# Samleo8/RadarSLAMPy

Measured on AMD Instinct MI355X. Metric: radar scan-pairs/sec (400x3768 polar), higher is better.
Workload: dtype u8/f32/f64

## Files before the change

### profiles/ri_prof.py

```python
#!/usr/bin/env python3
import ctypes as C, os, sys
sys.path.insert(0, os.path.dirname(os.path.dirname(os.path.abspath(__file__))))
import numpy as np
from radarslampy_amd import _ffi, synth
from radarslampy_amd.engine import Engine
os.environ["ROAM_LIB_PARTIAL"] = "1"
N = 512
recs, poses, feat = synth.make_sequence(5, 2, n_static=460, n_movers=24, distortion=True)
ctx = _ffi.Context(0)
eng = Engine(N, 2 * N, ctx=ctx, retrack_on_device=True, retrack_slots=N)
for t in range(2): eng.upload_scan(t, recs[t])
for b in range(1, N):
    for t in range(2): eng.copy_scan(b * 2 + t, t)
for b in range(N): eng.init_lane(b, b * 2, feat[:40], poses[0])
eng.set_retrack(2); eng.step(np.arange(N, dtype=np.int32) * 2 + 1); eng.synchronize()
lib = _ffi.load_library()
lib.roam_debug_integral_prof.argtypes = [C.c_void_p, C.c_int]
out = (C.c_ulonglong * 16)()
lib.roam_debug_integral_prof(out, 1)
ms, by = eng.time_kernel("doh_integral", 3)
lib.roam_debug_integral_prof(out, 0)
v = np.array(list(out), float)
names = ["col: loop head", "col: barrier wait", "col: C (tile -> HBM)", "col: A1 (box + taps)", "col: A2 (column sums -> tile)", "row: loop head", "row: barrier wait", "row: B = rest"]
print(f"doh_integral {ms:.2f} ms per {N}")
tot_c = v[:5].sum()
for k in range(5): print(f"  {names[k]:32s} {100 * v[k] / tot_c:5.1f} %")
tot_r = v[8 + 5] + v[8 + 6]
print(f"  row wave: loop body (B + head) {100 * v[8 + 5] / tot_r:5.1f} %   barrier wait {100 * v[8 + 6] / tot_r:5.1f} %")
eng.close(); ctx.close()
```

### radarslampy_amd/csrc/engine.hip

```cpp
#include "roam_internal.h"
#include "retrack.h"
#include "kabsch_body.inc"
#include <algorithm>
#include <new>

#define KS ROAM_MAX_FEATURES
#define CART_CENTER 1012.0
#define M_PER_PX 0.0864
#define N_RETRACK 60
#define ROT_THR 0.2
#define TRANS_THR_SQ 4.0
#define ERR_THR 10.0f
#define TWO_PI 6.283185307179586476925286766559

#define RES_RING 8
enum { ST_PEAKS = 0, ST_WARP, ST_PYR, ST_KLT, ST_GRAPH, ST_CLIQUE, ST_KABSCH, ST_LM, ST_GLUE, ST_RETRACK, ST_COUNT };
static const char *kStageNames[ST_COUNT] = {"ingest_peaks", "warp_quantise", "pyramid", "klt", "consistency_graph",
                                            "max_clique", "kabsch", "mds_lm", "glue", "retrack"};

struct Engine {
    roam_engine_cfg cfg;
    int B = 0, W = 0, stage_cap = 0;
    PyrDesc pd;
    size_t rec_bytes = 0;
// ... 691 lines not shown
            return ROAM_E_HIP;
        }
        RtArgs &r = e->rt;
        r.pool = e->pool; r.map = e->warp_map; r.feat = e->feat; r.feat_n = e->feat_n; r.vel = e->vel; r.kf_und = e->kf_und; r.res = nullptr;
    }
    for (auto &ev : e->ev_res)
        if (hipEventCreateWithFlags(&ev, hipEventDisableTiming) != hipSuccess) { ROAM_SET_ERR(ctx, "hipEventCreate failed"); roam_engine_destroy(ctx); return ROAM_E_HIP; }
    e->slot_seq.assign((size_t)cfg->pool_scans, 0);
    for (auto &ev : e->ev_up_ring)
        if (hipEventCreateWithFlags(&ev, hipEventDisableTiming) != hipSuccess) { ROAM_SET_ERR(ctx, "hipEventCreate failed"); roam_engine_destroy(ctx); return ROAM_E_HIP; }
    if (hipEventCreateWithFlags(&e->ev_pool, hipEventDisableTiming) != hipSuccess) {
        ROAM_SET_ERR(ctx, "hipEventCreate failed"); roam_engine_destroy(ctx); return ROAM_E_HIP;
    }
    for (auto &ev : e->ev) {
        if (hipEventCreate(&ev) != hipSuccess) { ROAM_SET_ERR(ctx, "hipEventCreate failed"); roam_engine_destroy(ctx); return ROAM_E_HIP; }
    }
    if (hipEventCreate(&e->ev_join) != hipSuccess ||
        hipEventCreate(&e->ev_pk0) != hipSuccess || hipEventCreate(&e->ev_pk1) != hipSuccess ||
        hipEventCreateWithFlags(&e->ev_warp, hipEventDisableTiming) != hipSuccess || hipEventCreateWithFlags(&e->ev_idx, hipEventDisableTiming) != hipSuccess ||
        hipEventCreateWithFlags(&e->ev_peaks, hipEventDisableTiming) != hipSuccess) {
        ROAM_SET_ERR(ctx, "hipEventCreate failed"); roam_engine_destroy(ctx); return ROAM_E_HIP;
    }
    for (int i = 0; i < 4; i++)
        if (hipEventCreateWithFlags(&e->ev_klt[i], hipEventDisableTiming) != hipSuccess || hipEventCreateWithFlags(&e->ev_g4[i], hipEventDisableTiming) != hipSuccess) {
            ROAM_SET_ERR(ctx, "hipEventCreate failed"); roam_engine_destroy(ctx); return ROAM_E_HIP;
        }
    e->ev_ok = true;
    e->tr_ok = true;
    HIP_TRY(ctx, launch_warp_map(ctx->stream, cfg->rows, cfg->clip, e->warp_map));
    HIP_TRY(ctx, launch_pyr_dark(ctx->stream, e->warp_map, e->W, e->W, cfg->clip, e->pyr_dark));
    if (e->rt_on) HIP_TRY(ctx, launch_retrack_boxtab(ctx->stream, e->warp_map, e->W, cfg->clip, const_cast<uint32_t *>(e->rt.boxtab)));
    if (e->rt_on) HIP_TRY(ctx, launch_retrack_darktab(ctx->stream, e->warp_map, e->W, cfg->clip, const_cast<uint32_t *>(e->rt.darktab)));
    if (e->rt_on && e->rt.fused) { const int32_t rc_ = fused_tables(ctx, e); if (rc_ != ROAM_OK) { roam_engine_destroy(ctx); return rc_; } }
    HIP_TRY(ctx, hipStreamSynchronize(ctx->stream));
    e->rt_image_px = (int64_t)e->W * e->W;
    if (e->rt_on && e->W <= 2048 && B >= RT_TWO_PASS_SLOTS) {
        e->rt_image_px = 0;
        const size_t npx = (size_t)e->W * e->W, ndt = retrack_darktab_words(e->W), nph = retrack_phase_words(e->W);
        uint32_t *stage = nullptr;
        HIP_TRY(ctx, hipHostMalloc(reinterpret_cast<void **>(&stage), (npx + ndt + nph) * 4, hipHostMallocDefault));
        uint32_t *mh = stage, *dh = stage + npx;
        std::vector<uint32_t> ph(nph, 0u);
        hipError_t ec = hipMemcpyAsync(mh, e->warp_map, npx * 4, hipMemcpyDeviceToHost, ctx->stream);
        if (ec == hipSuccess) ec = hipMemcpyAsync(dh, e->rt.darktab, ndt * 4, hipMemcpyDeviceToHost, ctx->stream);
        if (ec == hipSuccess) ec = hipStreamSynchronize(ctx->stream);
        bool okp = ec == hipSuccess && retrack_build_phases(mh, dh, e->W, cfg->clip, ph.data());
        if (okp) {
            memcpy(stage + npx + ndt, ph.data(), nph * 4);
            ec = hipMemcpyAsync(const_cast<uint32_t *>(e->rt.phlist), stage + npx + ndt, nph * 4, hipMemcpyHostToDevice, ctx->stream);
            if (ec == hipSuccess) ec = hipStreamSynchronize(ctx->stream);
        }
        (void)hipHostFree(stage);
        if (!okp || ec != hipSuccess) { ROAM_SET_ERR(ctx, "retrack: phase list (%s)", ec != hipSuccess ? hipGetErrorString(ec) : "image too large"); roam_engine_destroy(ctx); return ec != hipSuccess ? ROAM_E_HIP : ROAM_E_ARG; }
        for (uint32_t i = 0; i < ph[0]; i++) {
            const int br = retrack_band_rows(), band = (int)(ph[1 + i] & 255u), g = (int)((ph[1 + i] >> 8) & 15u), hrows = std::min(br, e->W - br * band);
            for (int w = 0; w < 4; w++)
                if ((ph[1 + i] >> (12 + w)) & 1u) e->rt_image_px += (int64_t)hrows * std::max(0, std::min(64, e->W - (g * 256 + 64 * w)));
        }
    }
    return ROAM_OK;
}

#define ENGINE()                                  \
    if (!ctx) return ROAM_E_ARG;                  \
    Engine *e = ctx->engine;                      \
    if (!e) { ROAM_SET_ERR(ctx, "engine not created"); return ROAM_E_STATE; } \
    HIP_TRY(ctx, hipSetDevice(ctx->device))

int32_t roam_engine_upload_scan(roam_ctx *ctx, int32_t pool_idx, const uint8_t *rec)
{
    ENGINE();
    ARG_CHECK(ctx, rec && pool_idx >= 0 && pool_idx < e->cfg.pool_scans);
    e->slot_writes[(size_t)pool_idx]++;
    HIP_TRY(ctx, hipMemcpyAsync(e->pool + (size_t)pool_idx * e->rec_bytes, rec, e->rec_bytes, hipMemcpyHostToDevice, ctx->stream));
    HIP_TRY(ctx, hipStreamSynchronize(ctx->stream));
    return ROAM_OK;
}

int32_t roam_engine_upload_scans_async(roam_ctx *ctx, int32_t pool_idx0, int32_t n, const uint8_t *host_records, int64_t host_stride)
{
    ENGINE();
    ARG_CHECK(ctx, host_records && n >= 1 && pool_idx0 >= 0 && pool_idx0 + n <= e->cfg.pool_scans && (host_stride == 0 || host_stride >= (int64_t)e->rec_bytes));
    hipPointerAttribute_t at;
    const hipError_t pa = hipPointerGetAttributes(&at, host_records);
    if (pa != hipSuccess || (at.type != hipMemoryTypeHost && at.type != hipMemoryTypeManaged && at.type != hipMemoryTypeDevice)) {
        (void)hipGetLastError();
        ROAM_SET_ERR(ctx, "upload_scans_async: host_records is not pinned host memory (hipHostMalloc / hipHostRegister / roam_host_alloc)");
        return ROAM_E_ARG;
    }
    const uint8_t *dev_alias = at.devicePointer ? static_cast<const uint8_t *>(at.devicePointer) : host_records;
    const int width = e->cfg.payload_off + e->cfg.clip;
    hipLaunchKernelGGL(ingest_rows_kernel, dim3((e->cfg.rows + 3) / 4, n), dim3(256), 0, ctx->stream3, dev_alias, host_stride,
                       e->pool + (size_t)pool_idx0 * e->rec_bytes, (int64_t)e->rec_bytes, e->cfg.rows, e->cfg.stride, width);
    HIP_TRY(ctx, hipGetLastError());
    HIP_TRY(ctx, hipEventRecord(ctx->ev_up, ctx->stream3));
    e->up_seq++;
    for (int i = 0; i < n; i++) { e->slot_seq[(size_t)pool_idx0 + i] = e->up_seq; e->slot_writes[(size_t)pool_idx0 + i]++; }
    HIP_TRY(ctx, hipEventRecord(e->ev_up_ring[e->up_seq & 15], ctx->stream3));
    e->uploads_pending = true;
    return ROAM_OK;
}

int32_t roam_engine_fence(roam_ctx *ctx)
{
    ENGINE();
    HIP_TRY(ctx, hipEventRecord(ctx->ev_fence, ctx->stream));
    HIP_TRY(ctx, hipStreamWaitEvent(ctx->stream3, ctx->ev_fence, 0));
    return ROAM_OK;
}

int32_t roam_engine_copy_scan(roam_ctx *ctx, int32_t dst_idx, int32_t src_idx)
// ... 1012 lines not shown
```

### radarslampy_amd/csrc/retrack.h

```cpp
#pragma once
#include "roam_internal.h"
#include "blobprune.h"

#define RT_TWO_PASS_SLOTS 200
enum { RT_F_CAND_OVERFLOW = 1, RT_F_TREE_OVERFLOW = 2, RT_F_PAIR_OVERFLOW = 4, RT_F_FEAT_OVERFLOW = 8 };

struct RtArgs {
    int W, rows, cols, stride, payload_off, slots, size1, size2;
    int64_t rec_bytes;
    double sigma1, sigma2, threshold;
    const uint8_t *pool;
    const uint32_t *map;
    const uint32_t *phlist;
    const uint32_t *boxtab;
    const uint32_t *darktab;
    float *feat;
    int32_t *feat_n;
    const double *vel;
    double *kf_und;
    roam_lane_result *res;
    int32_t *rt_n, *rt_lane, *rt_scan;
    double *S;
    int32_t *col_done;
    double *colT;
    int SP;
    uint32_t *cand_rc;
    double *cand_val;
    int32_t *cand_n;
    BpTask *tasks;
    uint32_t *pairs;
    uint16_t *order;
    uint32_t *ovbits;
    uint16_t *bigtab;
    double *kp;
    int32_t *kp_n, *slot_flags;
    int32_t *ssc_work;
    int32_t *sel, *sel_n;
    int32_t *blob_order_buf;
    const int32_t *blob_order;
    int fused;
    const uint32_t *fd_mapT;
    const uint32_t *fd_boxtab;
    const uint32_t *fd_darktab;
    double *fd_halo;
    int64_t fd_halo_words;
    double *fd_cc;
};

hipError_t launch_retrack_collect(hipStream_t st, const roam_lane_result *res, const int32_t *scan_idx, int B, int force_all, const RtArgs &a);
#define RT_TRACE_CHUNKS 16
struct RtSide { hipStream_t st; hipEvent_t ev_i[4], ev_d[4]; int chunk; };
bool retrack_sided(const RtArgs &a, int B, const RtSide *side);
hipError_t launch_retrack(hipStream_t st, const RtArgs &a, int B, hipEvent_t *trace = nullptr, int ntrace = 0, hipEvent_t after_order = nullptr, const RtSide *side = nullptr);
hipError_t launch_ssc_batch(hipStream_t st, const double *kp, int64_t kp_stride, const int32_t *count, int kp_cap, int P,
                            int num_ret, double tol, int cols, int rows, int32_t *work, int32_t *sel, int32_t *n_sel,
                            const int32_t *n_active, int first);
hipError_t launch_retrack_part(hipStream_t st, const RtArgs &a, int P, int which);
hipError_t launch_retrack_emit(hipStream_t st, const RtArgs &a, int P);
hipError_t retrack_init();
size_t retrack_boxtab_words(int W);
size_t retrack_phase_words(int W);
int retrack_band_rows();
bool retrack_build_phases(const uint32_t *map_host, const uint32_t *darktab_host, int W, int cols, uint32_t *out);
hipError_t launch_retrack_boxtab(hipStream_t st, const uint32_t *map, int W, int cols, uint32_t *boxtab);
size_t retrack_darktab_words(int W);
size_t retrack_fused_boxtab_words(int W);
size_t retrack_fused_halo_words(int W);
hipError_t launch_retrack_fused_tables(hipStream_t st, const uint32_t *map, int W, int cols, uint32_t *mapT, uint32_t *boxtab, uint32_t *darktab);
hipError_t launch_retrack_darktab(hipStream_t st, const uint32_t *map, int W, int cols, uint32_t *darktab);
```

### radarslampy_amd/csrc/retrack_integral.hip

```cpp
#include "retrack_geom.h"

#define RT_TWO_PASS_Z 8
#define RC_BAND 64
#define RC_Q 16
__global__ __launch_bounds__(256) void rt_integ_cols_kernel(RtArgs a, int first, int P)
{
    const int nls = rt_one_sweep(a, first) ? 0 : min(min(RT_TWO_PASS_SLOTS, P), *a.rt_n - first);
    if ((int)blockIdx.z >= nls) return;
    __shared__ double tot[4][64];
    __shared__ float lut[256];
    __shared__ int last_s;
    lut[threadIdx.x] = rt_code_to_f32(threadIdx.x);
    const int lane = threadIdx.x & 63, q = threadIdx.x >> 6;
    const int c = blockIdx.x * 64 + lane, W = a.W, band = blockIdx.y, nb = (W + RC_BAND - 1) / RC_BAND;
    for (int ls = blockIdx.z; ls < nls; ls += (int)gridDim.z) {
    const int slot = first + ls;
    const uint8_t *p = a.pool + (int64_t)a.rt_scan[slot] * a.rec_bytes + a.payload_off;
    double *S = a.S + (int64_t)ls * a.SP * W;
    const int rows = a.rows, cols = a.cols, stride = a.stride;
    const int r0 = band * RC_BAND + q * RC_Q;
    uint32_t m[RC_Q];
#pragma unroll
    for (int k = 0; k < RC_Q; k++) m[k] = (c < W && r0 + k < W) ? a.map[(int64_t)(r0 + k) * W + c] : 0xfffu;
    __syncthreads();
// ... 69 lines not shown
    double acc = 0;
    auto step = [&](double2 (&x)[8], double2 &o, int i) {
        const int c = i * RR_COLS + lc;
#pragma unroll
        for (int k = 0; k < 8; k++) {
            const bool rin = r0 + 2 * k + lr < H;
            *reinterpret_cast<double2 *>(&tile[2 * k + lr][lc]) =
                make_double2(rin && c < W ? __dadd_rn(x[k].x, o.x) : 0.0, rin && c + 1 < W ? __dadd_rn(x[k].y, o.y) : 0.0);
        }
        fetch(x, o, min(i + RR_DEPTH, ntiles - 1));
        __syncthreads();
        if (threadIdx.x < RR_ROWS) {
            double2 *row = reinterpret_cast<double2 *>(tile[threadIdx.x]);
            double2 y[8], z[8];
#pragma unroll
            for (int j = 0; j < 8; j++) y[j] = row[j];
            for (int j0 = 0; j0 < RR_COLS / 2; j0 += 16) {
#pragma unroll
                for (int j = 0; j < 8; j++) z[j] = row[j0 + 8 + j];
#pragma unroll
                for (int j = 0; j < 8; j++) { acc = __dadd_rn(acc, y[j].x); y[j].x = acc; acc = __dadd_rn(acc, y[j].y); y[j].y = acc; }
#pragma unroll
                for (int j = 0; j < 8; j++) row[j0 + j] = y[j];
                const int jn = min(j0 + 16, RR_COLS / 2 - 8);
#pragma unroll
                for (int j = 0; j < 8; j++) y[j] = row[jn + j];
#pragma unroll
                for (int j = 0; j < 8; j++) { acc = __dadd_rn(acc, z[j].x); z[j].x = acc; acc = __dadd_rn(acc, z[j].y); z[j].y = acc; }
#pragma unroll
                for (int j = 0; j < 8; j++) row[j0 + 8 + j] = z[j];
            }
        }
        __syncthreads();
#pragma unroll
        for (int k = 0; k < 8; k++) {
            const int r = r0 + 2 * k + lr;
            const double2 t2 = *reinterpret_cast<const double2 *>(&tile[2 * k + lr][lc]);
            if (r < H && c + 1 < W) *reinterpret_cast<double2 *>(S + (int64_t)r * a.SP + c) = t2;
            else if (r < H && c < W) S[(int64_t)r * a.SP + c] = t2.x;
        }
    };
    int i0 = 0;
    for (; i0 + RR_DEPTH <= ntiles; i0 += RR_DEPTH) {
#pragma unroll
        for (int d = 0; d < RR_DEPTH; d++) step(reg[d], off[d], i0 + d);
    }
#pragma unroll
    for (int d = 0; d < RR_DEPTH - 1; d++)
        if (i0 + d < ntiles) step(reg[d], off[d], i0 + d);
    __syncthreads();
    }
}

#ifndef RI_ROWS
#define RI_ROWS 16
#endif
#ifndef RI_WAVES
#define RI_WAVES 4
#endif
#define RI_GROUPS (2048 / (64 * RI_WAVES))
#define RI_PHL_MAX 1024
#ifndef RI_BD
#define RI_BD 4
#endif
#define RI_TP 66
#define RI_LDS_BYTES (2 * RI_WAVES * RI_ROWS * RI_TP * 8)
#ifndef RI_BOX
#define RI_BOX 2560
#endif
__global__ __launch_bounds__(64) void rt_boxtab_kernel(const uint32_t *__restrict__ map, int W, int cols, uint32_t *__restrict__ boxtab)
{
    const int H = W, lane = threadIdx.x;
    const int idx = blockIdx.x, wave = idx % RI_WAVES, g = (idx / RI_WAVES) % RI_GROUPS, band = idx / (RI_WAVES * RI_GROUPS);
    const int c = min(g * 64 * RI_WAVES + 64 * wave + lane, W - 1);
    int mnx = 0x7fffffff, mxx = -1, mny = 0x7fffffff, mxy = -1;
    for (int k = 0; k < RI_ROWS; k++) {
        const uint32_t m = map[(int64_t)min(band * RI_ROWS + k, H - 1) * W + c];
        const int ix = m & 4095, iy = (m >> 12) & 1023;
        if (ix < cols) { mnx = min(mnx, ix); mxx = max(mxx, ix); mny = min(mny, iy); mxy = max(mxy, iy); }
    }
    for (int d = 32; d >= 1; d >>= 1) {
        mnx = min(mnx, __shfl_xor(mnx, d)); mxx = max(mxx, __shfl_xor(mxx, d));
        mny = min(mny, __shfl_xor(mny, d)); mxy = max(mxy, __shfl_xor(mxy, d));
    }
    if (lane == 0) {
        boxtab[2 * idx] = mxx < 0 ? 0xffff0000u : ((uint32_t)mnx | ((uint32_t)mxx << 16));
        boxtab[2 * idx + 1] = mxx < 0 ? 0u : ((uint32_t)mny | ((uint32_t)mxy << 16));
    }
}

#ifdef RI_PROF
__device__ unsigned long long ri_prof[16];
extern "C" int roam_debug_integral_prof(unsigned long long *out, int reset)
{
    if (hipMemcpyFromSymbol(out, HIP_SYMBOL(ri_prof), sizeof(ri_prof)) != hipSuccess) return -1;
    if (reset) { unsigned long long z[16] = {0}; if (hipMemcpyToSymbol(HIP_SYMBOL(ri_prof), z, sizeof(z)) != hipSuccess) return -1; }
    return 0;
}
#define RI_P(k) { const unsigned long long tn_ = __builtin_amdgcn_s_memtime(); rip_[k] += tn_ - rit_; rit_ = tn_; }
#else
#define RI_P(k)
#endif
__global__ __launch_bounds__(64 * (RI_WAVES + 1)) void rt_integral_kernel(RtArgs a, int first)
{
#ifdef RI_PROF
    unsigned long long rip_[8] = {0}, rit_ = __builtin_amdgcn_s_memtime();
#endif
    extern __shared__ __align__(16) double ri_lds[];
    const int ls = (int)blockIdx.x, slot = first + ls;
    if (slot >= *a.rt_n || !rt_one_sweep(a, first) || a.fused) return;
    typedef double Tile[RI_ROWS][RI_TP];
    Tile *tiles = reinterpret_cast<Tile *>(ri_lds);
    const int W = a.W, H = a.W, t = threadIdx.x, wave = t >> 6, lane = t & 63;
    __shared__ float lut[256];
    __shared__ __align__(4) uint8_t box[RI_WAVES][RI_BOX];
    __shared__ uint16_t phl[RI_PHL_MAX];
    if (t < 256) lut[t] = rt_code_to_f32(t);
    const int nph = (int)a.phlist[0];
    for (int i = t; i < nph; i += (int)blockDim.x) phl[i] = (uint16_t)a.phlist[1 + i];
    __syncthreads();
    auto ph_ent = [&](int i) { return i < nph ? (int)__builtin_amdgcn_readfirstlane((int)phl[i]) : 0; };
    auto ph_band = [](int e) { return e & 255; };
    auto ph_group = [](int e) { return (e >> 8) & 15; };
    if (wave < RI_WAVES) {
        const uint8_t *p = a.pool + (int64_t)a.rt_scan[slot] * a.rec_bytes + a.payload_off;
        double *S = a.S + (int64_t)ls * a.SP * W;
        const int SP = a.SP;
        const int rows = a.rows, cols = a.cols, stride = a.stride;
        double acc[RI_GROUPS];
#pragma unroll
        for (int g = 0; g < RI_GROUPS; g++) acc[g] = 0.0;
        uint32_t m[RI_ROWS];
        uint32_t ext0 = 0, ext1 = 0;
        uint32_t cur0 = 0xffff0000u, cur1 = 0;
        uint32_t raw[8];
        const int wave_u = __builtin_amdgcn_readfirstlane(wave);
        auto fetch = [&](int band, int g) {
            const int c = min(g * 64 * RI_WAVES + 64 * wave + lane, W - 1);
#pragma unroll
            for (int k = 0; k < RI_ROWS; k++) m[k] = a.map[(int64_t)min(band * RI_ROWS + k, H - 1) * W + c];
        };
        auto fetch_ext = [&](int i) {
            const uint32_t *bt = a.boxtab + 2 * (i * RI_WAVES + wave_u);
            ext0 = bt[0]; ext1 = bt[1];
        };
        struct Box { int mnx, mxx, mny, mxy, bh, bp, nrg, ncb; bool staged, inside; };
        auto geom = [&](uint32_t e0, uint32_t e1) {
            Box b;
            b.mnx = e0 & 0xffff; b.mxx = (e0 >> 16) == 0xffff ? -1 : (int)(e0 >> 16); b.mny = e1 & 0xffff; b.mxy = e1 >> 16;
            const int bw = b.mxx - b.mnx + 2;
            b.bh = b.mxy - b.mny + 2; b.bp = (bw + 3) & ~3;
            b.nrg = (b.bh + 3) >> 2; b.ncb = (b.bp + 63) >> 6;
            b.staged = b.mxx >= 0 && b.bp * b.bh <= RI_BOX && cols >= 4;
            b.inside = b.staged && b.mny >= 1 && b.mny - 1 + 4 * b.nrg <= rows && b.mnx + 64 * b.ncb <= cols;
            return b;
        };
        const int sub = lane >> 4, c4 = (lane & 15) * 4;
        auto load_pieces = [&](const Box &b, int q0) {
            const uint8_t *pl = p + (sub * stride + c4);
            const int npiece = b.nrg * b.ncb;
            int kg = (q0 / b.ncb) * 4, cb = (q0 % b.ncb) * 64;
#pragma unroll
            for (int u = 0; u < 8; u++) {
                if (q0 + u < npiece) raw[u] = reinterpret_cast<const RtU32 *>(pl + ((b.mny - 1 + kg) * stride + b.mnx + cb))->v;
                cb += 64;
                if (cb >= b.bp) { cb = 0; kg += 4; }
            }
        };
        auto store_pieces = [&](const Box &b, int q0, uint8_t *bx) {
            uint8_t *bl = bx + (sub * b.bp + c4);
            const int npiece = b.nrg * b.ncb;
            int kg = (q0 / b.ncb) * 4, cb = (q0 % b.ncb) * 64;
#pragma unroll
            for (int u = 0; u < 8; u++) {
                if (q0 + u < npiece && sub < b.bh - kg && c4 < b.bp - cb) *reinterpret_cast<uint32_t *>(bl + (kg * b.bp + cb)) = raw[u];
                cb += 64;
                if (cb >= b.bp) { cb = 0; kg += 4; }
            }
        };
        auto prefetch_box = [&]() {
            cur0 = __builtin_amdgcn_readfirstlane(ext0); cur1 = __builtin_amdgcn_readfirstlane(ext1);
            const Box b = geom(cur0, cur1);
            if (b.inside) load_pieces(b, 0);
        };
        float v[RI_ROWS];
        auto A1 = [&](int i, int e_n1, int e_n2) {
            const Box b = geom(cur0, cur1);
            const int mnx = b.mnx, mny = b.mny, bh = b.bh, bp = b.bp;
            if (b.mxx < 0) {
#pragma unroll
                for (int k = 0; k < RI_ROWS; k++) v[k] = 0.f;
            } else if (b.staged) {
                uint8_t *bx = box[wave];
                if (b.inside) {
                    const int npiece = b.nrg * b.ncb;
                    for (int q0 = 0; q0 < npiece; q0 += 8) {
                        if (q0 > 0) load_pieces(b, q0);
                        store_pieces(b, q0, bx);
                    }
                } else
                for (int kg = 0; kg < bh; kg += 4) {
                    const int kk = kg + sub;
                    int r = mny + kk - 1;
                    if (r < 0) r += rows; else if (r >= rows) r -= rows;
                    for (int cb = 0; cb < bp; cb += 64) {
                        const int cc = cb + c4;
                        if (kk < bh && cc < bp) {
                            const int x0 = mnx + cc, xl = min(x0, cols - 4), sh = 8 * (x0 - xl);
                            uint32_t rw = 0;
                            if (sh < 32) rw = reinterpret_cast<const RtU32 *>(p + r * stride + xl)->v >> sh;
                            *reinterpret_cast<uint32_t *>(bx + kk * bp + cc) = rw;
                        }
                    }
                }
#pragma unroll
                for (int k = 0; k < RI_ROWS; k++) {
                    const uint32_t mk = m[k];
                    const int ix = mk & 4095, iy = (mk >> 12) & 1023;
                    float r_ = 0.f;
                    if (ix < cols) {
                        const float wx1 = __fmul_rn((float)((mk >> 22) & 31), 1.f / 32.f), wx0 = __fsub_rn(1.f, wx1);
                        const float wy1 = __fmul_rn((float)(mk >> 27), 1.f / 32.f), wy0 = __fsub_rn(1.f, wy1);
                        const uint8_t *q = bx + (iy - mny) * bp + (ix - mnx);
                        const float s00 = lut[q[0]], s01 = lut[q[1]], s10 = lut[q[bp]], s11 = lut[q[bp + 1]];
                        r_ = __fmul_rn(s00, __fmul_rn(wy0, wx0));
                        r_ = __fadd_rn(r_, __fmul_rn(s01, __fmul_rn(wy0, wx1)));
                        r_ = __fadd_rn(r_, __fmul_rn(s10, __fmul_rn(wy1, wx0)));
                        r_ = __fadd_rn(r_, __fmul_rn(s11, __fmul_rn(wy1, wx1)));
                    }
                    v[k] = r_;
                }
            } else {
#pragma unroll
                for (int k = 0; k < RI_ROWS; k++) v[k] = rt_pixel(m[k], p, rows, cols, stride, lut);
            }
            if (i + 1 < nph) {
                fetch(ph_band(e_n1), ph_group(e_n1));
                prefetch_box();
                if (i + 2 < nph) fetch_ext(ph_band(e_n2) * RI_GROUPS + ph_group(e_n2));
            }
        };
        int gcur = 0;
        auto A2 = [&](int i, int band, int g) {
            const int c = g * 64 * RI_WAVES + 64 * wave + lane;
            Tile &tl = tiles[(i & 1) * RI_WAVES + wave];
            {
                while (gcur != g) {
                    const double s0 = acc[0];
#pragma unroll
                    for (int q = 0; q + 1 < RI_GROUPS; q++) acc[q] = acc[q + 1];
                    acc[RI_GROUPS - 1] = s0;
                    gcur = (gcur + 1) % RI_GROUPS;
                }
                double s = acc[0];
                if (c < W) {
#pragma unroll
                    for (int k = 0; k < RI_ROWS; k++) {
                        if (band * RI_ROWS + k < H) s = __dadd_rn(s, (double)v[k]);
                        tl[k][lane] = s;
                    }
                }
#pragma unroll
                for (int q = 0; q + 1 < RI_GROUPS; q++) acc[q] = acc[q + 1];
                acc[RI_GROUPS - 1] = s;
                gcur = (gcur + 1) % RI_GROUPS;
            }
        };
        auto C = [&](int i, int e) {
            const int band = ph_band(e), g = ph_group(e);
            const int c = g * 64 * RI_WAVES + 64 * wave + lane;
            const Tile &tl = tiles[(i & 1) * RI_WAVES + wave];
            const bool wanted = ((e >> (12 + wave_u)) & 1) != 0;
            if (c < W && wanted) {
                double *q = S + (int64_t)band * RI_ROWS * SP + c;
                const int nk = min(RI_ROWS, H - band * RI_ROWS);
                if (nk == RI_ROWS) {
#pragma unroll
                    for (int k = 0; k < RI_ROWS; k++) q[(int64_t)k * SP] = tl[k][lane];
                } else
                    for (int k = 0; k < nk; k++) q[(int64_t)k * SP] = tl[k][lane];
            }
        };
        int e_m1 = 0, e_0 = ph_ent(0), e_1 = ph_ent(1), e_2 = ph_ent(2), e_3 = ph_ent(3);
        if (nph > 0) {
            fetch(ph_band(e_0), ph_group(e_0));
            fetch_ext(ph_band(e_0) * RI_GROUPS + ph_group(e_0));
            prefetch_box();
            if (nph > 1) fetch_ext(ph_band(e_1) * RI_GROUPS + ph_group(e_1));
            A1(0, e_1, e_2);
            A2(0, ph_band(e_0), ph_group(e_0));
#pragma unroll 1
            for (int i = 0; i < nph; i++) {
                const int e_4 = ph_ent(i + 4);
                RI_P(0)
                __syncthreads();
                RI_P(1)
                if (i > 0) C(i - 1, e_m1);
                RI_P(2)
                if (i + 1 < nph) { A1(i + 1, e_2, e_3); RI_P(3) A2(i + 1, ph_band(e_1), ph_group(e_1)); }
                RI_P(4)
                e_m1 = e_0; e_0 = e_1; e_1 = e_2; e_2 = e_3; e_3 = e_4;
            }
        }
        __syncthreads();
        if (nph > 0) C(nph - 1, e_m1);
    } else {
        double carry = 0.0;
        int pband = -1;
        int e_nx = ph_ent(0);
        for (int i = 0; i < nph; i++) {
            const int band = ph_band(e_nx), g = ph_group(e_nx);
            e_nx = ph_ent(i + 1);
            if (band != pband) { carry = 0.0; pband = band; }
            const bool live = lane < RI_ROWS && band * RI_ROWS + lane < H;
            RI_P(5)
            __syncthreads();
            RI_P(6)
            if (live) {
                const int C0 = g * 64 * RI_WAVES, ncols = min(64 * RI_WAVES, W - C0);
                Tile *tg = tiles + (i & 1) * RI_WAVES;
                int j = 0;
                if (ncols >= 16) {
                    auto rd = [&](double(&x)[8], int jj) {
                        const double2 *q = reinterpret_cast<const double2 *>(&tg[jj >> 6][lane][jj & 63]);
#pragma unroll
                        for (int u = 0; u < 4; u++) { const double2 v2 = q[u]; x[2 * u] = v2.x; x[2 * u + 1] = v2.y; }
                    };
                    auto chain_wr = [&](double(&x)[8], int jj) {
#pragma unroll
                        for (int u = 0; u < 8; u++) { carry = __dadd_rn(carry, x[u]); x[u] = carry; }
                        double2 *q = reinterpret_cast<double2 *>(&tg[jj >> 6][lane][jj & 63]);
#pragma unroll
                        for (int u = 0; u < 4; u++) q[u] = make_double2(x[2 * u], x[2 * u + 1]);
                    };
                    double xr[RI_BD][8];
#pragma unroll
                    for (int u = 0; u < RI_BD; u++)
                        if (8 * u + 8 <= ncols) rd(xr[u], 8 * u);
                    for (; j + 8 * RI_BD <= ncols; j += 8 * RI_BD) {
#pragma unroll
                        for (int u = 0; u < RI_BD; u++) {
                            chain_wr(xr[u], j + 8 * u);
                            if (j + 8 * (RI_BD + u) + 8 <= ncols) rd(xr[u], j + 8 * (RI_BD + u));
                        }
                    }
#pragma unroll
                    for (int u = 0; u < RI_BD; u++)
                        if (j + 8 <= ncols) { chain_wr(xr[u], j); j += 8; }
                }
                for (; j < ncols; j++) {
                    double *q = &tg[j >> 6][lane][j & 63];
                    carry = __dadd_rn(carry, *q);
                    *q = carry;
                }
            }
        }
        __syncthreads();
    }
#ifdef RI_PROF
    if (lane == 0 && (wave == 0 || wave == RI_WAVES)) for (int k = 0; k < 8; k++) atomicAdd(&ri_prof[k + (wave == 0 ? 0 : 8)], rip_[k]);
#endif
}

size_t retrack_boxtab_words(int W) { return 2 * (size_t)((W + RI_ROWS - 1) / RI_ROWS) * RI_GROUPS * RI_WAVES; }

hipError_t launch_retrack_boxtab(hipStream_t st, const uint32_t *map, int W, int cols, uint32_t *boxtab)
{
    hipLaunchKernelGGL(rt_boxtab_kernel, dim3((unsigned)(retrack_boxtab_words(W) / 2)), dim3(64), 0, st, map, W, cols, boxtab);
    return hipGetLastError();
}
size_t retrack_phase_words(int W) { return 1 + (size_t)((W + RI_ROWS - 1) / RI_ROWS) * RI_GROUPS; }
int retrack_band_rows() { return RI_ROWS; }

bool retrack_build_phases(const uint32_t *map, const uint32_t *darktab, int W, int cols, uint32_t *out)
{
    const int H = W, nbands = (H + RI_ROWS - 1) / RI_ROWS, ns = (W + SD_OUT - 1) / SD_OUT, nt = H / SD_T + 1, NT = RI_GROUPS * RI_WAVES;
    static_assert(RI_ROWS % SD_T == 0, "a band of the integral kernel is one or more blocks of the determinant kernel");
    const int ndet = (H + SD_T - 1) / SD_T;
    if (nbands * RI_GROUPS > RI_PHL_MAX || nbands > 256) return false;
    std::vector<uint8_t> need((size_t)nbands * NT, 0), lit((size_t)nbands * NT, 0);
    std::vector<int> firstlit(W, H);
    for (int r = 0; r < H; r++)
        for (int c = 0; c < W; c++)
            if ((int)(map[(size_t)r * W + c] & 4095u) < cols) {
                lit[(size_t)(r / RI_ROWS) * NT + c / 64] = 1;
                if (firstlit[c] == H) firstlit[c] = r;
            }
    for (int s = 0; s < ns; s++) {
        const uint32_t *T = darktab + (size_t)s * SD_DT_WORDS;
        const int t_first = (int)T[16], t_last = (int)T[17];
        if (t_first >= nt) continue;
        const int tb = t_first >= 1 ? ((t_first - 1) & ~3) : 0, te = std::min(nt, t_last + 2);
        const int cbase = s * SD_OUT - 1 - SD_HL, c_lo = std::max(cbase, 0), c_hi = std::min(cbase + SD_BP, W) - 1;
        for (int j = tb; j <= te + 3 && j < ndet; j++) {
            const bool in_loop = j >= tb + 4;
            if (in_loop && ((T[8 + ((j - 4) >> 5)] >> ((j - 4) & 31)) & 1u)) continue;
            for (int k = c_lo / 64; k <= c_hi / 64; k++) need[(size_t)(j * SD_T / RI_ROWS) * NT + k] = 1;
        }
    }
    int n = 0;
    bool sound = true;
    for (int b = 0; b < nbands; b++) {
        bool needp[RI_GROUPS], zero[RI_GROUPS];
        uint32_t bits[RI_GROUPS];
        for (int g = 0; g < RI_GROUPS; g++) {
            bits[g] = 0; zero[g] = true;
            for (int w = 0; w < RI_WAVES; w++) if (need[(size_t)b * NT + g * RI_WAVES + w]) bits[g] |= 1u << w;
            needp[g] = bits[g] != 0;
            const int rend = std::min(b * RI_ROWS + RI_ROWS - 1, H - 1);
            for (int c = g * 64 * RI_WAVES; c < std::min(W, (g + 1) * 64 * RI_WAVES); c++) if (firstlit[c] <= rend) { zero[g] = false; break; }
        }
        for (int g = 0; g < RI_GROUPS; g++) {
            bool skipL = !needp[g], skipR = true;
            for (int q = 0; q <= g && skipL; q++) skipL = zero[q];
            for (int q = g; q < RI_GROUPS && skipR; q++) skipR = !needp[q];
            if (g * 64 * RI_WAVES >= W) continue;
            if (skipL || skipR) {
                for (int w = 0; w < RI_WAVES; w++) if (lit[(size_t)b * NT + g * RI_WAVES + w]) sound = false;
                continue;
            }
            out[1 + n++] = (uint32_t)b | ((uint32_t)g << 8) | (bits[g] << 12);
        }
    }
    if (!sound) {
        n = 0;
        for (int b = 0; b < nbands; b++)
            for (int g = 0; g < RI_GROUPS && g * 64 * RI_WAVES < W; g++) out[1 + n++] = (uint32_t)b | ((uint32_t)g << 8) | (((1u << RI_WAVES) - 1u) << 12);
    }
    out[0] = (uint32_t)n;
    return true;
}

hipError_t retrack_integral_init() { return hipFuncSetAttribute(reinterpret_cast<const void *>(rt_integral_kernel), hipFuncAttributeMaxDynamicSharedMemorySize, RI_LDS_BYTES); }

hipError_t launch_retrack_integral(hipStream_t st, const RtArgs &a, int first, int P, bool one_sweep)
{
    if (one_sweep) hipLaunchKernelGGL(rt_integral_kernel, dim3(P), dim3(64 * (RI_WAVES + 1)), RI_LDS_BYTES, st, a, first);
    if (hipError_t e = hipGetLastError(); e != hipSuccess) return e;
    const int W = a.W, P2 = min(P, RT_TWO_PASS_SLOTS);
    hipLaunchKernelGGL(rt_integ_cols_kernel, dim3((W + 63) / 64, (W + RC_BAND - 1) / RC_BAND, min(P2, RT_TWO_PASS_Z)), dim3(256), 0, st, a, first, P2);
    hipLaunchKernelGGL(rt_integ_rows_kernel, dim3((W + RR_ROWS - 1) / RR_ROWS, min(P2, RT_TWO_PASS_Z)), dim3(256), 0, st, a, first, P2);
    return hipGetLastError();
}
```

Measured before the change: 53920.

## Restructure integral-image kernel: 64-row bands split into wave quarters per column tile

Changes the one-sweep integral kernel so that each phase covers one 64-column tile over a 64-row band. The four waves each take a quarter of the rows and combine their partial sums through LDS, where before each wave owned its own column group over 16-row bands. The phase list is now read through constant address space instead of being copied to LDS. HBM write-out of finished tiles moves to the row wave as coalesced double2 stores, overlapping with the column waves. Boxtab, phase building and pixel accounting are redone for the new layout. The changes aim for fewer phases and barriers, better store coalescing and two workgroups per CU, at the cost of cross-wave LDS reductions.

```diff
diff --git a/profiles/ri_prof.py b/profiles/ri_prof.py
--- a/profiles/ri_prof.py
+++ b/profiles/ri_prof.py
@@ -21,10 +21,10 @@
 ms, by = eng.time_kernel("doh_integral", 3)
 lib.roam_debug_integral_prof(out, 0)
 v = np.array(list(out), float)
-names = ["col: loop head", "col: barrier wait", "col: C (tile -> HBM)", "col: A1 (box + taps)", "col: A2 (column sums -> tile)", "row: loop head", "row: barrier wait", "row: B = rest"]
+names = ["col: loop head", "col: barrier wait", "col: A2 (base + column sums -> tile)", "col: A1 (box + taps + quarter total)"]
 print(f"doh_integral {ms:.2f} ms per {N}")
-tot_c = v[:5].sum()
-for k in range(5): print(f"  {names[k]:32s} {100 * v[k] / tot_c:5.1f} %")
-tot_r = v[8 + 5] + v[8 + 6]
-print(f"  row wave: loop body (B + head) {100 * v[8 + 5] / tot_r:5.1f} %   barrier wait {100 * v[8 + 6] / tot_r:5.1f} %")
+tot_c = v[:4].sum()
+for k in range(4): print(f"  {names[k]:32s} {100 * v[k] / tot_c:5.1f} %")
+tot_r = v[8 + 5] + v[8 + 6] + v[8 + 7]
+print(f"  row wave: B (the chain) {100 * v[8 + 7] / tot_r:5.1f} %   C (tile -> HBM) + loop head {100 * v[8 + 5] / tot_r:5.1f} %   barrier wait {100 * v[8 + 6] / tot_r:5.1f} %")
 eng.close(); ctx.close()
diff --git a/radarslampy_amd/csrc/engine.hip b/radarslampy_amd/csrc/engine.hip
--- a/radarslampy_amd/csrc/engine.hip
+++ b/radarslampy_amd/csrc/engine.hip
@@ -767,11 +767,7 @@
         }
         (void)hipHostFree(stage);
         if (!okp || ec != hipSuccess) { ROAM_SET_ERR(ctx, "retrack: phase list (%s)", ec != hipSuccess ? hipGetErrorString(ec) : "image too large"); roam_engine_destroy(ctx); return ec != hipSuccess ? ROAM_E_HIP : ROAM_E_ARG; }
-        for (uint32_t i = 0; i < ph[0]; i++) {
-            const int br = retrack_band_rows(), band = (int)(ph[1 + i] & 255u), g = (int)((ph[1 + i] >> 8) & 15u), hrows = std::min(br, e->W - br * band);
-            for (int w = 0; w < 4; w++)
-                if ((ph[1 + i] >> (12 + w)) & 1u) e->rt_image_px += (int64_t)hrows * std::max(0, std::min(64, e->W - (g * 256 + 64 * w)));
-        }
+        e->rt_image_px = retrack_phase_pixels(ph.data(), e->W);
     }
     return ROAM_OK;
 }
diff --git a/radarslampy_amd/csrc/retrack.h b/radarslampy_amd/csrc/retrack.h
--- a/radarslampy_amd/csrc/retrack.h
+++ b/radarslampy_amd/csrc/retrack.h
@@ -62,6 +62,7 @@
 size_t retrack_phase_words(int W);
 int retrack_band_rows();
 bool retrack_build_phases(const uint32_t *map_host, const uint32_t *darktab_host, int W, int cols, uint32_t *out);
+int64_t retrack_phase_pixels(const uint32_t *phases_host, int W);
 hipError_t launch_retrack_boxtab(hipStream_t st, const uint32_t *map, int W, int cols, uint32_t *boxtab);
 size_t retrack_darktab_words(int W);
 size_t retrack_fused_boxtab_words(int W);
diff --git a/radarslampy_amd/csrc/retrack_integral.hip b/radarslampy_amd/csrc/retrack_integral.hip
--- a/radarslampy_amd/csrc/retrack_integral.hip
+++ b/radarslampy_amd/csrc/retrack_integral.hip
@@ -145,30 +145,27 @@
     }
 }
 
-#ifndef RI_ROWS
-#define RI_ROWS 16
-#endif
-#ifndef RI_WAVES
+#define RI_ROWS 64
 #define RI_WAVES 4
-#endif
-#define RI_GROUPS (2048 / (64 * RI_WAVES))
-#define RI_PHL_MAX 1024
+#define RI_Q (RI_ROWS / RI_WAVES)
+#define RI_TILES (2048 / 64)
+#define RI_OWN (RI_TILES / RI_WAVES)
 #ifndef RI_BD
 #define RI_BD 4
 #endif
 #define RI_TP 66
-#define RI_LDS_BYTES (2 * RI_WAVES * RI_ROWS * RI_TP * 8)
-#ifndef RI_BOX
-#define RI_BOX 2560
-#endif
+#define RI_LDS_BYTES (2 * RI_ROWS * RI_TP * 8)
+#define RI_BOX 2048
+static_assert(RI_LDS_BYTES + 2 * RI_WAVES * 64 * 8 + 2 * 64 * 8 + RI_WAVES * RI_BOX + 256 * 4 <= 81920, "two workgroups per CU");
 __global__ __launch_bounds__(64) void rt_boxtab_kernel(const uint32_t *__restrict__ map, int W, int cols, uint32_t *__restrict__ boxtab)
 {
     const int H = W, lane = threadIdx.x;
-    const int idx = blockIdx.x, wave = idx % RI_WAVES, g = (idx / RI_WAVES) % RI_GROUPS, band = idx / (RI_WAVES * RI_GROUPS);
-    const int c = min(g * 64 * RI_WAVES + 64 * wave + lane, W - 1);
+    const int idx = blockIdx.x, tile = idx % RI_TILES, quarter = idx / RI_TILES;
+    const int c = min(tile * 64 + lane, W - 1);
     int mnx = 0x7fffffff, mxx = -1, mny = 0x7fffffff, mxy = -1;
-    for (int k = 0; k < RI_ROWS; k++) {
-        const uint32_t m = map[(int64_t)min(band * RI_ROWS + k, H - 1) * W + c];
+    for (int k = 0; k < RI_Q; k++) {
+        if (quarter * RI_Q + k >= H) break;
+        const uint32_t m = map[(int64_t)(quarter * RI_Q + k) * W + c];
         const int ix = m & 4095, iy = (m >> 12) & 1023;
         if (ix < cols) { mnx = min(mnx, ix); mxx = max(mxx, ix); mny = min(mny, iy); mxy = max(mxy, iy); }
     }
@@ -181,6 +178,11 @@
         boxtab[2 * idx + 1] = mxx < 0 ? 0u : ((uint32_t)mny | ((uint32_t)mxy << 16));
     }
 }
+
+#define RI_E_BAND(e) ((int)((e) & 63u))
+#define RI_E_TILE(e) ((int)(((e) >> 8) & 31u))
+#define RI_E_BITS(e) ((uint32_t)(((e) >> 16) & 15u))
+#define RI_E_MAKE(band, tile, bits) ((uint32_t)(band) | ((uint32_t)(tile) << 8) | ((uint32_t)(bits) << 16))
 
 #ifdef RI_PROF
 __device__ unsigned long long ri_prof[16];
@@ -207,34 +209,35 @@
     const int W = a.W, H = a.W, t = threadIdx.x, wave = t >> 6, lane = t & 63;
     __shared__ float lut[256];
     __shared__ __align__(4) uint8_t box[RI_WAVES][RI_BOX];
-    __shared__ uint16_t phl[RI_PHL_MAX];
+    __shared__ double tot[2][RI_WAVES][64];
+    __shared__ double cb[2][64];
     if (t < 256) lut[t] = rt_code_to_f32(t);
-    const int nph = (int)a.phlist[0];
-    for (int i = t; i < nph; i += (int)blockDim.x) phl[i] = (uint16_t)a.phlist[1 + i];
-    __syncthreads();
-    auto ph_ent = [&](int i) { return i < nph ? (int)__builtin_amdgcn_readfirstlane((int)phl[i]) : 0; };
-    auto ph_band = [](int e) { return e & 255; };
-    auto ph_group = [](int e) { return (e >> 8) & 15; };
+    typedef const uint32_t __attribute__((address_space(4))) *RiConstPtr;
+    const RiConstPtr phc = (RiConstPtr)(uintptr_t)a.phlist;
+    const int nph = (int)phc[0];
+    auto ph_ent = [&](int i) { return i < nph ? phc[1 + i] : 0u; };
+    __syncthreads();
     if (wave < RI_WAVES) {
         const uint8_t *p = a.pool + (int64_t)a.rt_scan[slot] * a.rec_bytes + a.payload_off;
         double *S = a.S + (int64_t)ls * a.SP * W;
         const int SP = a.SP;
         const int rows = a.rows, cols = a.cols, stride = a.stride;
-        double acc[RI_GROUPS];
-#pragma unroll
-        for (int g = 0; g < RI_GROUPS; g++) acc[g] = 0.0;
-        uint32_t m[RI_ROWS];
+        const int wave_u = __builtin_amdgcn_readfirstlane(wave);
+        double own[RI_OWN];
+#pragma unroll
+        for (int g = 0; g < RI_OWN; g++) own[g] = 0.0;
+        int gcur = 0;
+        uint32_t m[RI_Q];
         uint32_t ext0 = 0, ext1 = 0;
         uint32_t cur0 = 0xffff0000u, cur1 = 0;
         uint32_t raw[8];
-        const int wave_u = __builtin_amdgcn_readfirstlane(wave);
-        auto fetch = [&](int band, int g) {
-            const int c = min(g * 64 * RI_WAVES + 64 * wave + lane, W - 1);
-#pragma unroll
-            for (int k = 0; k < RI_ROWS; k++) m[k] = a.map[(int64_t)min(band * RI_ROWS + k, H - 1) * W + c];
-        };
-        auto fetch_ext = [&](int i) {
-            const uint32_t *bt = a.boxtab + 2 * (i * RI_WAVES + wave_u);
+        auto fetch = [&](uint32_t e) {
+            const int c = min(RI_E_TILE(e) * 64 + lane, W - 1), r0 = RI_E_BAND(e) * RI_ROWS + wave_u * RI_Q;
+#pragma unroll
+            for (int k = 0; k < RI_Q; k++) m[k] = a.map[(int64_t)min(r0 + k, H - 1) * W + c];
+        };
+        auto fetch_ext = [&](uint32_t e) {
+            const uint32_t *bt = a.boxtab + 2 * ((RI_E_BAND(e) * RI_WAVES + wave_u) * RI_TILES + RI_E_TILE(e));
             ext0 = bt[0]; ext1 = bt[1];
         };
         struct Box { int mnx, mxx, mny, mxy, bh, bp, nrg, ncb; bool staged, inside; };
@@ -252,23 +255,23 @@
         auto load_pieces = [&](const Box &b, int q0) {
             const uint8_t *pl = p + (sub * stride + c4);
             const int npiece = b.nrg * b.ncb;
-            int kg = (q0 / b.ncb) * 4, cb = (q0 % b.ncb) * 64;
+            int kg = (q0 / b.ncb) * 4, cb_ = (q0 % b.ncb) * 64;
 #pragma unroll
             for (int u = 0; u < 8; u++) {
-                if (q0 + u < npiece) raw[u] = reinterpret_cast<const RtU32 *>(pl + ((b.mny - 1 + kg) * stride + b.mnx + cb))->v;
-                cb += 64;
-                if (cb >= b.bp) { cb = 0; kg += 4; }
+                if (q0 + u < npiece) raw[u] = reinterpret_cast<const RtU32 *>(pl + ((b.mny - 1 + kg) * stride + b.mnx + cb_))->v;
+                cb_ += 64;
+                if (cb_ >= b.bp) { cb_ = 0; kg += 4; }
             }
         };
         auto store_pieces = [&](const Box &b, int q0, uint8_t *bx) {
             uint8_t *bl = bx + (sub * b.bp + c4);
             const int npiece = b.nrg * b.ncb;
-            int kg = (q0 / b.ncb) * 4, cb = (q0 % b.ncb) * 64;
+            int kg = (q0 / b.ncb) * 4, cb_ = (q0 % b.ncb) * 64;
 #pragma unroll
             for (int u = 0; u < 8; u++) {
-                if (q0 + u < npiece && sub < b.bh - kg && c4 < b.bp - cb) *reinterpret_cast<uint32_t *>(bl + (kg * b.bp + cb)) = raw[u];
-                cb += 64;
-                if (cb >= b.bp) { cb = 0; kg += 4; }
+                if (q0 + u < npiece && sub < b.bh - kg && c4 < b.bp - cb_) *reinterpret_cast<uint32_t *>(bl + (kg * b.bp + cb_)) = raw[u];
+                cb_ += 64;
+                if (cb_ >= b.bp) { cb_ = 0; kg += 4; }
             }
         };
         auto prefetch_box = [&]() {
@@ -276,13 +279,23 @@
             const Box b = geom(cur0, cur1);
             if (b.inside) load_pieces(b, 0);
         };
-        float v[RI_ROWS];
-        auto A1 = [&](int i, int e_n1, int e_n2) {
+        float v[RI_Q];
+        double vtot = 0.0;
+        auto rotate_to = [&](int g) {
+            while (gcur != g) {
+                const double s0 = own[0];
+#pragma unroll
+                for (int q = 0; q + 1 < RI_OWN; q++) own[q] = own[q + 1];
+                own[RI_OWN - 1] = s0;
+                gcur = (gcur + 1) % RI_OWN;
+            }
+        };
+        auto A1 = [&](int i, uint32_t e_i, uint32_t e_n1, uint32_t e_n2) {
             const Box b = geom(cur0, cur1);
             const int mnx = b.mnx, mny = b.mny, bh = b.bh, bp = b.bp;
             if (b.mxx < 0) {
 #pragma unroll
-                for (int k = 0; k < RI_ROWS; k++) v[k] = 0.f;
+                for (int k = 0; k < RI_Q; k++) v[k] = 0.f;
             } else if (b.staged) {
                 uint8_t *bx = box[wave];
                 if (b.inside) {
@@ -296,8 +309,8 @@
                     const int kk = kg + sub;
                     int r = mny + kk - 1;
                     if (r < 0) r += rows; else if (r >= rows) r -= rows;
-                    for (int cb = 0; cb < bp; cb += 64) {
-                        const int cc = cb + c4;
+                    for (int cb_ = 0; cb_ < bp; cb_ += 64) {
+                        const int cc = cb_ + c4;
                         if (kk < bh && cc < bp) {
                             const int x0 = mnx + cc, xl = min(x0, cols - 4), sh = 8 * (x0 - xl);
                             uint32_t rw = 0;
@@ -307,7 +320,7 @@
                     }
                 }
 #pragma unroll
-                for (int k = 0; k < RI_ROWS; k++) {
+                for (int k = 0; k < RI_Q; k++) {
                     const uint32_t mk = m[k];
                     const int ix = mk & 4095, iy = (mk >> 12) & 1023;
                     float r_ = 0.f;
@@ -325,104 +338,95 @@
                 }
             } else {
 #pragma unroll
-                for (int k = 0; k < RI_ROWS; k++) v[k] = rt_pixel(m[k], p, rows, cols, stride, lut);
+                for (int k = 0; k < RI_Q; k++) v[k] = rt_pixel(m[k], p, rows, cols, stride, lut);
             }
             if (i + 1 < nph) {
-                fetch(ph_band(e_n1), ph_group(e_n1));
+                fetch(e_n1);
                 prefetch_box();
-                if (i + 2 < nph) fetch_ext(ph_band(e_n2) * RI_GROUPS + ph_group(e_n2));
-            }
-        };
-        int gcur = 0;
-        auto A2 = [&](int i, int band, int g) {
-            const int c = g * 64 * RI_WAVES + 64 * wave + lane;
-            Tile &tl = tiles[(i & 1) * RI_WAVES + wave];
-            {
-                while (gcur != g) {
-                    const double s0 = acc[0];
-#pragma unroll
-                    for (int q = 0; q + 1 < RI_GROUPS; q++) acc[q] = acc[q + 1];
-                    acc[RI_GROUPS - 1] = s0;
-                    gcur = (gcur + 1) % RI_GROUPS;
-                }
-                double s = acc[0];
-                if (c < W) {
-#pragma unroll
-                    for (int k = 0; k < RI_ROWS; k++) {
-                        if (band * RI_ROWS + k < H) s = __dadd_rn(s, (double)v[k]);
-                        tl[k][lane] = s;
-                    }
-                }
-#pragma unroll
-                for (int q = 0; q + 1 < RI_GROUPS; q++) acc[q] = acc[q + 1];
-                acc[RI_GROUPS - 1] = s;
-                gcur = (gcur + 1) % RI_GROUPS;
-            }
-        };
-        auto C = [&](int i, int e) {
-            const int band = ph_band(e), g = ph_group(e);
-            const int c = g * 64 * RI_WAVES + 64 * wave + lane;
-            const Tile &tl = tiles[(i & 1) * RI_WAVES + wave];
-            const bool wanted = ((e >> (12 + wave_u)) & 1) != 0;
-            if (c < W && wanted) {
-                double *q = S + (int64_t)band * RI_ROWS * SP + c;
-                const int nk = min(RI_ROWS, H - band * RI_ROWS);
-                if (nk == RI_ROWS) {
-#pragma unroll
-                    for (int k = 0; k < RI_ROWS; k++) q[(int64_t)k * SP] = tl[k][lane];
-                } else
-                    for (int k = 0; k < nk; k++) q[(int64_t)k * SP] = tl[k][lane];
-            }
-        };
-        int e_m1 = 0, e_0 = ph_ent(0), e_1 = ph_ent(1), e_2 = ph_ent(2), e_3 = ph_ent(3);
+                if (i + 2 < nph) fetch_ext(e_n2);
+            }
+            const int nlive = H - (RI_E_BAND(e_i) * RI_ROWS + wave_u * RI_Q);
+            double s = 0.0;
+#pragma unroll
+            for (int k = 0; k < RI_Q; k++) {
+                if (k >= nlive) v[k] = 0.f;
+                s = __dadd_rn(s, (double)v[k]);
+            }
+            vtot = s;
+            tot[i & 1][wave][lane] = s;
+            if ((RI_E_TILE(e_i) & (RI_WAVES - 1)) == wave_u) {
+                rotate_to(RI_E_TILE(e_i) / RI_WAVES);
+                cb[i & 1][lane] = own[0];
+            }
+        };
+        auto A2 = [&](int i, uint32_t e_i) {
+            const bool owner = (RI_E_TILE(e_i) & (RI_WAVES - 1)) == wave_u;
+            double s = cb[i & 1][lane], sum = vtot;
+#pragma unroll
+            for (int q = 0; q < RI_WAVES; q++) {
+                if (q == wave_u || !(q < wave_u || owner)) continue;
+                const double tq = tot[i & 1][q][lane];
+                if (q < wave_u) s = __dadd_rn(s, tq);
+                sum = __dadd_rn(sum, tq);
+            }
+            if (owner) own[0] = __dadd_rn(own[0], sum);
+            double (*tl)[RI_TP] = tiles[i & 1] + wave * RI_Q;
+#pragma unroll
+            for (int k = 0; k < RI_Q; k++) {
+                s = __dadd_rn(s, (double)v[k]);
+                tl[k][lane] = s;
+            }
+        };
+        uint32_t e_0 = ph_ent(0), e_1 = ph_ent(1), e_2 = ph_ent(2), e_3 = ph_ent(3);
         if (nph > 0) {
-            fetch(ph_band(e_0), ph_group(e_0));
-            fetch_ext(ph_band(e_0) * RI_GROUPS + ph_group(e_0));
+            fetch(e_0);
+            fetch_ext(e_0);
             prefetch_box();
-            if (nph > 1) fetch_ext(ph_band(e_1) * RI_GROUPS + ph_group(e_1));
-            A1(0, e_1, e_2);
-            A2(0, ph_band(e_0), ph_group(e_0));
+            if (nph > 1) fetch_ext(e_1);
+            A1(0, e_0, e_1, e_2);
+        }
 #pragma unroll 1
-            for (int i = 0; i < nph; i++) {
-                const int e_4 = ph_ent(i + 4);
-                RI_P(0)
-                __syncthreads();
-                RI_P(1)
-                if (i > 0) C(i - 1, e_m1);
-                RI_P(2)
-                if (i + 1 < nph) { A1(i + 1, e_2, e_3); RI_P(3) A2(i + 1, ph_band(e_1), ph_group(e_1)); }
-                RI_P(4)
-                e_m1 = e_0; e_0 = e_1; e_1 = e_2; e_2 = e_3; e_3 = e_4;
-            }
-        }
-        __syncthreads();
-        if (nph > 0) C(nph - 1, e_m1);
+        for (int i = 0; i < nph + 1; i++) {
+            const uint32_t e_4 = ph_ent(i + 4);
+            RI_P(0)
+            __syncthreads();
+            RI_P(1)
+            if (i < nph) A2(i, e_0);
+            RI_P(2)
+            if (i + 1 < nph) A1(i + 1, e_1, e_2, e_3);
+            RI_P(3)
+            e_0 = e_1; e_1 = e_2; e_2 = e_3; e_3 = e_4;
+        }
     } else {
+        double *S = a.S + (int64_t)ls * a.SP * W;
+        const int SP = a.SP;
+        const int half = lane >> 5, c2 = 2 * (lane & 31);
         double carry = 0.0;
         int pband = -1;
-        int e_nx = ph_ent(0);
-        for (int i = 0; i < nph; i++) {
-            const int band = ph_band(e_nx), g = ph_group(e_nx);
-            e_nx = ph_ent(i + 1);
-            if (band != pband) { carry = 0.0; pband = band; }
-            const bool live = lane < RI_ROWS && band * RI_ROWS + lane < H;
+        uint32_t e_nx = ph_ent(0);
+        for (int i = 0; i < nph + 1; i++) {
+            const uint32_t e = e_nx;
+            if (i >= 1) e_nx = ph_ent(i);
             RI_P(5)
             __syncthreads();
             RI_P(6)
-            if (live) {
-                const int C0 = g * 64 * RI_WAVES, ncols = min(64 * RI_WAVES, W - C0);
-                Tile *tg = tiles + (i & 1) * RI_WAVES;
+            if (i < 1) continue;
+            const int band = RI_E_BAND(e), tile = RI_E_TILE(e);
+            if (band != pband) { carry = 0.0; pband = band; }
+            if (band * RI_ROWS + lane < H) {
+                const int ncols = min(64, W - tile * 64);
+                double *row = tiles[(i - 1) & 1][lane];
                 int j = 0;
                 if (ncols >= 16) {
                     auto rd = [&](double(&x)[8], int jj) {
-                        const double2 *q = reinterpret_cast<const double2 *>(&tg[jj >> 6][lane][jj & 63]);
+                        const double2 *q = reinterpret_cast<const double2 *>(row + jj);
 #pragma unroll
                         for (int u = 0; u < 4; u++) { const double2 v2 = q[u]; x[2 * u] = v2.x; x[2 * u + 1] = v2.y; }
                     };
                     auto chain_wr = [&](double(&x)[8], int jj) {
 #pragma unroll
                         for (int u = 0; u < 8; u++) { carry = __dadd_rn(carry, x[u]); x[u] = carry; }
-                        double2 *q = reinterpret_cast<double2 *>(&tg[jj >> 6][lane][jj & 63]);
+                        double2 *q = reinterpret_cast<double2 *>(row + jj);
 #pragma unroll
                         for (int u = 0; u < 4; u++) q[u] = make_double2(x[2 * u], x[2 * u + 1]);
                     };
@@ -442,41 +446,53 @@
                         if (j + 8 <= ncols) { chain_wr(xr[u], j); j += 8; }
                 }
                 for (; j < ncols; j++) {
-                    double *q = &tg[j >> 6][lane][j & 63];
-                    carry = __dadd_rn(carry, *q);
-                    *q = carry;
+                    carry = __dadd_rn(carry, row[j]);
+                    row[j] = carry;
                 }
             }
-        }
-        __syncthreads();
+            RI_P(7)
+            if (tile * 64 + c2 < W) {
+                const double (*tl)[RI_TP] = tiles[(i - 1) & 1];
+                double *q = S + (int64_t)(band * RI_ROWS + half) * SP + tile * 64 + c2;
+                for (int w = 0; w < RI_WAVES; w++) {
+                    if (!((RI_E_BITS(e) >> w) & 1u)) continue;
+                    double2 x[RI_Q / 2];
+#pragma unroll
+                    for (int k = 0; k < RI_Q / 2; k++) x[k] = *reinterpret_cast<const double2 *>(&tl[w * RI_Q + 2 * k + half][c2]);
+#pragma unroll
+                    for (int k = 0; k < RI_Q / 2; k++)
+                        if (band * RI_ROWS + w * RI_Q + 2 * k + half < H) *reinterpret_cast<double2 *>(q + (int64_t)(w * RI_Q + 2 * k) * SP) = x[k];
+                }
+            }
+        }
     }
 #ifdef RI_PROF
     if (lane == 0 && (wave == 0 || wave == RI_WAVES)) for (int k = 0; k < 8; k++) atomicAdd(&ri_prof[k + (wave == 0 ? 0 : 8)], rip_[k]);
 #endif
 }
 
-size_t retrack_boxtab_words(int W) { return 2 * (size_t)((W + RI_ROWS - 1) / RI_ROWS) * RI_GROUPS * RI_WAVES; }
+size_t retrack_boxtab_words(int W) { return 2 * (size_t)((W + RI_ROWS - 1) / RI_ROWS) * RI_WAVES * RI_TILES; }
 
 hipError_t launch_retrack_boxtab(hipStream_t st, const uint32_t *map, int W, int cols, uint32_t *boxtab)
 {
     hipLaunchKernelGGL(rt_boxtab_kernel, dim3((unsigned)(retrack_boxtab_words(W) / 2)), dim3(64), 0, st, map, W, cols, boxtab);
     return hipGetLastError();
 }
-size_t retrack_phase_words(int W) { return 1 + (size_t)((W + RI_ROWS - 1) / RI_ROWS) * RI_GROUPS; }
+size_t retrack_phase_words(int W) { return 1 + (size_t)((W + RI_ROWS - 1) / RI_ROWS) * RI_TILES; }
 int retrack_band_rows() { return RI_ROWS; }
 
 bool retrack_build_phases(const uint32_t *map, const uint32_t *darktab, int W, int cols, uint32_t *out)
 {
-    const int H = W, nbands = (H + RI_ROWS - 1) / RI_ROWS, ns = (W + SD_OUT - 1) / SD_OUT, nt = H / SD_T + 1, NT = RI_GROUPS * RI_WAVES;
-    static_assert(RI_ROWS % SD_T == 0, "a band of the integral kernel is one or more blocks of the determinant kernel");
+    const int H = W, nbands = (H + RI_ROWS - 1) / RI_ROWS, ns = (W + SD_OUT - 1) / SD_OUT, nt = H / SD_T + 1, NT = RI_TILES;
+    static_assert(RI_ROWS % SD_T == 0 && RI_Q % SD_T == 0, "a quarter of a band of the integral kernel is one or more blocks of the determinant kernel");
     const int ndet = (H + SD_T - 1) / SD_T;
-    if (nbands * RI_GROUPS > RI_PHL_MAX || nbands > 256) return false;
-    std::vector<uint8_t> need((size_t)nbands * NT, 0), lit((size_t)nbands * NT, 0);
+    if (W > 64 * RI_TILES) return false;
+    std::vector<uint8_t> need((size_t)nbands * RI_WAVES * NT, 0), lit((size_t)nbands * RI_WAVES * NT, 0);
     std::vector<int> firstlit(W, H);
     for (int r = 0; r < H; r++)
         for (int c = 0; c < W; c++)
             if ((int)(map[(size_t)r * W + c] & 4095u) < cols) {
-                lit[(size_t)(r / RI_ROWS) * NT + c / 64] = 1;
+                lit[(size_t)(r / RI_Q) * NT + c / 64] = 1;
                 if (firstlit[c] == H) firstlit[c] = r;
             }
     for (int s = 0; s < ns; s++) {
@@ -488,40 +504,55 @@
         for (int j = tb; j <= te + 3 && j < ndet; j++) {
             const bool in_loop = j >= tb + 4;
             if (in_loop && ((T[8 + ((j - 4) >> 5)] >> ((j - 4) & 31)) & 1u)) continue;
-            for (int k = c_lo / 64; k <= c_hi / 64; k++) need[(size_t)(j * SD_T / RI_ROWS) * NT + k] = 1;
-        }
-    }
+            for (int k = c_lo / 64; k <= c_hi / 64; k++) need[(size_t)(j * SD_T / RI_Q) * NT + k] = 1;
+        }
+    }
+    const int ntile = (W + 63) / 64;
     int n = 0;
     bool sound = true;
     for (int b = 0; b < nbands; b++) {
-        bool needp[RI_GROUPS], zero[RI_GROUPS];
-        uint32_t bits[RI_GROUPS];
-        for (int g = 0; g < RI_GROUPS; g++) {
-            bits[g] = 0; zero[g] = true;
-            for (int w = 0; w < RI_WAVES; w++) if (need[(size_t)b * NT + g * RI_WAVES + w]) bits[g] |= 1u << w;
-            needp[g] = bits[g] != 0;
-            const int rend = std::min(b * RI_ROWS + RI_ROWS - 1, H - 1);
-            for (int c = g * 64 * RI_WAVES; c < std::min(W, (g + 1) * 64 * RI_WAVES); c++) if (firstlit[c] <= rend) { zero[g] = false; break; }
-        }
-        for (int g = 0; g < RI_GROUPS; g++) {
-            bool skipL = !needp[g], skipR = true;
-            for (int q = 0; q <= g && skipL; q++) skipL = zero[q];
-            for (int q = g; q < RI_GROUPS && skipR; q++) skipR = !needp[q];
-            if (g * 64 * RI_WAVES >= W) continue;
+        bool zero[RI_TILES];
+        uint32_t bits[RI_TILES];
+        const int rend = std::min(b * RI_ROWS + RI_ROWS - 1, H - 1);
+        for (int k = 0; k < ntile; k++) {
+            bits[k] = 0; zero[k] = true;
+            for (int w = 0; w < RI_WAVES; w++) if (need[(size_t)(b * RI_WAVES + w) * NT + k]) bits[k] |= 1u << w;
+            for (int c = k * 64; c < std::min(W, (k + 1) * 64); c++) if (firstlit[c] <= rend) { zero[k] = false; break; }
+        }
+        for (int k = 0; k < ntile; k++) {
+            bool skipL = !bits[k], skipR = true;
+            for (int q = 0; q <= k && skipL; q++) skipL = zero[q];
+            for (int q = k; q < ntile && skipR; q++) skipR = !bits[q];
             if (skipL || skipR) {
-                for (int w = 0; w < RI_WAVES; w++) if (lit[(size_t)b * NT + g * RI_WAVES + w]) sound = false;
+                for (int w = 0; w < RI_WAVES; w++) if (lit[(size_t)(b * RI_WAVES + w) * NT + k]) sound = false;
                 continue;
             }
-            out[1 + n++] = (uint32_t)b | ((uint32_t)g << 8) | (bits[g] << 12);
+            out[1 + n++] = RI_E_MAKE(b, k, bits[k]);
         }
     }
     if (!sound) {
         n = 0;
         for (int b = 0; b < nbands; b++)
-            for (int g = 0; g < RI_GROUPS && g * 64 * RI_WAVES < W; g++) out[1 + n++] = (uint32_t)b | ((uint32_t)g << 8) | (((1u << RI_WAVES) - 1u) << 12);
+            for (int k = 0; k < ntile; k++) {
+                uint32_t all = 0;
+                for (int w = 0; w < RI_WAVES; w++) if (b * RI_ROWS + w * RI_Q < H) all |= 1u << w;
+                out[1 + n++] = RI_E_MAKE(b, k, all);
+            }
     }
     out[0] = (uint32_t)n;
     return true;
+}
+
+int64_t retrack_phase_pixels(const uint32_t *ph, int W)
+{
+    int64_t px = 0;
+    for (uint32_t i = 0; i < ph[0]; i++) {
+        const uint32_t e = ph[1 + i];
+        const int wcols = std::max(0, std::min(64, W - RI_E_TILE(e) * 64));
+        for (int w = 0; w < RI_WAVES; w++)
+            if ((RI_E_BITS(e) >> w) & 1u) px += (int64_t)std::max(0, std::min(RI_Q, W - (RI_E_BAND(e) * RI_ROWS + w * RI_Q))) * wcols;
+    }
+    return px;
 }
 
 hipError_t retrack_integral_init() { return hipFuncSetAttribute(reinterpret_cast<const void *>(rt_integral_kernel), hipFuncAttributeMaxDynamicSharedMemorySize, RI_LDS_BYTES); }
```

Result: faster. 57080, median of 6 (+5.9%).
